# ZhenlongYuan/DVP-MVS

Hardware: AMD Instinct MI355X
Metric: Mpixels/sec/PatchMatch-iteration (higher is better)
Workload: dtype f32

## Files before the change

__graft_entry__.py:

```python
import importlib
import os
import subprocess
import sys

ROOT = os.path.dirname(os.path.abspath(__file__))
if ROOT not in sys.path:
    sys.path.insert(0, ROOT)


def build() -> None:
    subprocess.check_call(["make", "-s", "-C", os.path.join(ROOT, "dvp-mvs_amd", "csrc")])
    host = os.path.join(ROOT, "dvp-mvs_amd", "host")
    if os.path.exists(os.path.join(host, "Makefile")):
        subprocess.check_call(["make", "-s", "-C", host])
    subprocess.check_call(["make", "-s", "-C", os.path.join(ROOT, "oracle")])
    subprocess.check_call(["make", "-s", "-C", os.path.join(ROOT, "tests", "emul")])
    subprocess.check_call(["make", "-s", "-C", os.path.join(ROOT, "tests", "host")])
    subprocess.check_call(["make", "-s", "-C", os.path.join(ROOT, "tests", "half16")])
    subprocess.check_call(["make", "-s", "-C", os.path.join(ROOT, "tests", "jpeg_host")])
    pkg = importlib.import_module("dvp-mvs_amd")
    lib = pkg.get_capi().lib()
    missing = [s for s in pkg.get_capi().EXPORTS if not hasattr(lib, s)]
    if missing:
        raise RuntimeError("libdvp_mvs_hip.so lacks symbols: %s" % missing)


def smoke() -> None:
    import numpy as np
    pkg = importlib.import_module("dvp-mvs_amd")
    synth, capi = pkg.synth, pkg.get_capi()
    from oracle import oracle as O
    W, H, S = 96, 64, 3
    sc = synth.make_scene(W, H, S)
    p = synth.default_params(S + 1, max_iterations=1, state=synth.FIRST_INIT, use_APD=0)
    p["depth_min"] = np.float32(2.5) * np.float32(0.6)
    p["depth_max"] = np.float32(6.5) * np.float32(1.2)
    state = dict(planes=np.zeros((H * W, 4), np.float32), edge=sc["edge"], label=sc["label"],
                 radius=np.full(H * W, 5, np.int32))
    g = capi.from_scene(sc, p, device=0)
    g.upload_state(**state)
    g.run_patchmatch()
    o = O.from_scene(sc, p)
    o.upload_state(**state)
    o.run_patchmatch()
    pg, po = g.get("planes"), o.get("planes")
    same = (pg.view(np.uint32) == po.view(np.uint32)) | (np.isnan(pg) & np.isnan(po))
    if not same.all():
        raise AssertionError("smoke: HIP planes differ from the oracle in %d values" % int((~same).sum()))
    for n in ("selected_views", "weak_info", "radius"):
        if not (g.get(n) == o.get(n)).all():
            raise AssertionError("smoke: %s differs from the oracle" % n)
    print("smoke ok: %dx%d S=%d bit-exact vs oracle; total %.2f ms" % (W, H, S, g.timings()["total_ms"]))


if __name__ == "__main__":
    build()
    if os.path.exists("/dev/kfd"):
        smoke()
```

dvp-mvs_amd/csrc/dvp_engine.hip:

```cpp
#include "dvp_stages.hpp"
#include "dvp_jpeg_enc.h"
#include <hip/hip_runtime.h>
#include <cstdlib>
#include <string>
#include <vector>
#include <cstdio>
#include <cstring>
#include <mutex>
#include <condition_variable>
#include <thread>
#include <chrono>
#include <algorithm>
#include <cmath>

using namespace dvp;

struct LaunchArgs {
	int tiles_x, tiles, rows, half, colour, iter;
};

template <int STAGE, int SMP, int MV = 32>
__device__ __forceinline__ void stage_body(const Dev& d, const LaunchArgs& a) {
	const int lane = threadIdx.x & 63;
	const int wave = threadIdx.x >> 6;
// ... 140 lines not shown
	for (int i0 = 0; i0 < total; i0 += 64) {
		const bool valid = i0 + lane < total;
		const int i = valid ? i0 + lane : total - 1;
		const int pl = items[i];
		const int k = i - __shfl(off, pl, 64);
		uint32_t m = (uint32_t)__shfl((int)uniq, pl, 64);
		for (int j = 0; j < k; ++j) m &= m - 1;
		const int slot = dvp_ctz(m);
		PatchCtx ci;
		ci.tab = PatchTab{&lds_tab[pl], 64};
		ci.sum_ref = __shfl(c.sum_ref, pl, 64);
		ci.sum_ref_ref = __shfl(c.sum_ref_ref, pl, 64);
		ci.wsum = __shfl(c.wsum, pl, 64);
		ci.radius = __shfl(c.radius, pl, 64);
		ci.inc = __shfl(c.inc, pl, 64);
		ci.fast = __shfl(c.fast, pl, 64);
		const int ipx = __shfl(px, pl, 64), ipy = __shfl(py, pl, 64);
		strong_eval_item<SMP>(d, ci, ipx, ipy, slot, valid, d.eval_counter ? &cnt : nullptr);
	}
	if (d.eval_counter && cnt) atomicAdd(d.eval_counter, cnt);
}
extern "C" __global__ void __launch_bounds__(64, DVP_LB_HEAVY) dvp_strong_eval_items(const Dev d, const LaunchArgs a) { strong_eval_items_body<0>(d, a); }
extern "C" __global__ void __launch_bounds__(64, DVP_LB_HEAVY) dvp_strong_eval_items_exact(const Dev d, const LaunchArgs a) { strong_eval_items_body<1>(d, a); }
DVP_KERNEL64(dvp_strong_refine, kStageStrongRefine, DVP_LB_HEAVY)
DVP_KERNEL64(dvp_strong_refine_lanes, kStageStrongRefineLanes, DVP_LB_HEAVY)
template <int MV>
__device__ __forceinline__ void strong_decide_body(const Dev& d, const LaunchArgs& a) {
	int px, py;
	if (!block_to_pixel(blockIdx.x, threadIdx.x & 63, threadIdx.x >> 6, a.tiles_x, a.tiles, a.rows, a.half, a.colour, d.width, d.height, &px, &py)) return;
	if (d.weak_info[px + py * d.width] != DVP_WEAK) strong_decide_px<MV>(d, px, py, a.iter);
}
#ifndef DVP_LB_DECIDE
#define DVP_LB_DECIDE 4
#endif
#define DVP_DECIDE_KERNEL(MV) extern "C" __global__ void __launch_bounds__(256, DVP_LB_DECIDE) dvp_strong_decide_v##MV(const Dev d, const LaunchArgs a) { strong_decide_body<MV>(d, a); }
DVP_DECIDE_KERNEL(4)
DVP_DECIDE_KERNEL(6)
DVP_DECIDE_KERNEL(8)
DVP_DECIDE_KERNEL(10)
DVP_DECIDE_KERNEL(12)
DVP_DECIDE_KERNEL(16)
DVP_KERNEL(dvp_get_depth_normal, DVP_ST_GET_DEPTH_NORMAL, 1)
DVP_KERNEL(dvp_filter_strong, DVP_ST_FILTER_STRONG, 1)
DVP_KERNEL(dvp_depth_to_weak, DVP_ST_DEPTH_TO_WEAK, DVP_LB_HEAVY)
DVP_KERNEL(dvp_local_refine, DVP_ST_LOCAL_REFINE, DVP_LB_HEAVY)
DVP_KERNEL(dvp_depth_to_weak_refine, kStageSweeps, DVP_LB_HEAVY)
template <int WHAT>
__device__ __forceinline__ void sweep_light_body(const Dev& d, const LaunchArgs& a) {
	int px, py;
	if (!block_to_pixel(blockIdx.x, threadIdx.x & 63, threadIdx.x >> 6, a.tiles_x, a.tiles, a.rows, 0, 0, d.width, d.height, &px, &py)) return;
	if (WHAT != 0 && d.sweep_row1 > 0 && (py < d.sweep_row0 || py >= d.sweep_row1)) return;
	if (WHAT == 0) sweep_prepare_px(d, px, py);
	else if (WHAT == 1) sweep_decide1_px(d, px, py);
	else sweep_decide2_px(d, px, py);
}
extern "C" __global__ void __launch_bounds__(256) dvp_sweep_prepare(const Dev d, const LaunchArgs a) { sweep_light_body<0>(d, a); }
extern "C" __global__ void __launch_bounds__(256) dvp_sweep_decide1(const Dev d, const LaunchArgs a) { sweep_light_body<1>(d, a); }
extern "C" __global__ void __launch_bounds__(256) dvp_sweep_decide2(const Dev d, const LaunchArgs a) { sweep_light_body<2>(d, a); }
#ifndef DVP_SWEEP_ROWS
#define DVP_SWEEP_ROWS 14
#endif
constexpr int kSweepRows = DVP_SWEEP_ROWS;
template <int SMP>
__device__ __forceinline__ void sweep_eval_body(const Dev& d, const LaunchArgs& a) {
	const int lane = threadIdx.x;
	const int v = blockIdx.y;
	__shared__ f2 lds_tab[kTaps * kTaps * 64];
	__shared__ uint16_t list[64 * kSweepRows];
	__shared__ DvpCamera cams[2];
	const PatchTab tab{&lds_tab[lane], 64};
	static_assert(sizeof(DvpCamera) == 112, "28 dwords");
	if (lane < 56) {
		const int which = lane >= 28 ? 1 : 0;
		reinterpret_cast<uint32_t*>(&cams[which])[lane - 28 * which] = reinterpret_cast<const uint32_t*>(d.cameras + (which ? v + 1 : 0))[lane - 28 * which];
	}
	const int tiles_y = a.tiles / a.tiles_x;
	int tx, ty;
	{
		const int per_strip = 8 * tiles_y;
		const int st = (int)blockIdx.x / per_strip, rem = (int)blockIdx.x - st * per_strip;
		const int w_last = a.tiles_x - st * 8;
		if (w_last >= 8) { ty = rem >> 3; tx = st * 8 + (rem & 7); }
		else { ty = rem / w_last; tx = st * 8 + (rem - ty * w_last); }
	}
	ty += a.rows;
	const int x = tx * 64 + lane;
	int n = 0;
	for (int r = 0; r < kSweepRows; ++r) {
		const int y = ty * kSweepRows + r;
		const bool go = x < d.width && y < d.height && sweep_go(d, x + y * d.width, v, a.iter);
		const unsigned long long m = __ballot(go);
		if (go) list[n + __popcll(m & ((1ull << lane) - 1ull))] = (uint16_t)(r * 64 + lane);
		n += __popcll(m);
	}
	__syncthreads();
	unsigned long long cnt = 0;
	for (int i0 = 0; i0 < n; i0 += 64) {
		if (i0 + lane < n) {
			const int e = list[i0 + lane];
			sweep_eval_px<SMP>(d, tx * 64 + (e & 63), ty * kSweepRows + (e >> 6), v, a.iter, tab, d.eval_counter ? &cnt : nullptr, cams);
		}
	}
	if (d.eval_counter && cnt) atomicAdd(d.eval_counter, cnt);
}
template <int SMP>
__device__ __forceinline__ void sweep_border_body(const Dev& d, const LaunchArgs& a) {
	__shared__ f2 lds_tab[kTaps * kTaps * 64];
	const PatchTab tab{&lds_tab[threadIdx.x], 64};
	const int W = d.width, H = d.height;
	const long long t = (long long)blockIdx.x * 64 + threadIdx.x;
	int px, py;
	if (t < 12ll * W) {
		const int r = (int)(t / W);
		px = (int)(t - (long long)r * W);
		py = r < 6 ? r : H - 12 + r;
	} else {
		const long long u = t - 12ll * W;
		const int r = (int)(u / 12), cidx = (int)(u - 12ll * r);
		if (r >= H - 12) return;
		py = 6 + r;
		px = cidx < 6 ? cidx : W - 12 + cidx;
	}
	unsigned long long n = 0;
	run_pixel<kStageSweeps, SMP>(d, px, py, kSweepBorderOnly, d.eval_counter ? &n : nullptr, tab);
	if (d.eval_counter && n) atomicAdd(d.eval_counter, n);
}
extern "C" __global__ void __launch_bounds__(64, DVP_LB_HEAVY) dvp_sweep_border(const Dev d, const LaunchArgs a) { sweep_border_body<0>(d, a); }
extern "C" __global__ void __launch_bounds__(64, DVP_LB_HEAVY) dvp_sweep_border_exact(const Dev d, const LaunchArgs a) { sweep_border_body<1>(d, a); }
extern "C" __global__ void __launch_bounds__(64, DVP_LB_HEAVY) dvp_sweep_eval(const Dev d, const LaunchArgs a) { sweep_eval_body<0>(d, a); }
extern "C" __global__ void __launch_bounds__(64, DVP_LB_HEAVY) dvp_sweep_eval_exact(const Dev d, const LaunchArgs a) { sweep_eval_body<1>(d, a); }

DVP_KERNEL_LIST(dvp_find_nearest_strong_list, DVP_ST_FIND_NEAREST_STRONG, 1)
extern "C" __global__ void __launch_bounds__(256) dvp_gen_neighbours_list(const Dev d, const ListArgs a) {
	__shared__ s2 pts[kGnDirSlots * 256];
	const int t = list_block(blockIdx.x, gridDim.x, kListRun) * 256 + threadIdx.x;
	if (t >= a.count) return;
	const int center = d.weak_list[a.base + t];
	const int py = center / d.width, px = center - py * d.width;
	gen_neighbours_px(d, px, py, pts + threadIdx.x, 256);
}
DVP_KERNEL_LIST(dvp_neighbour_update_list, DVP_ST_NEIGHBOUR_UPDATE, 1)
DVP_KERNEL_LIST(dvp_ransac_fit_plane_list, DVP_ST_RANSAC_FIT, 1)
extern "C" __global__ void __launch_bounds__(64) dvp_ransac_fit_plane_wave(const Dev d, const ListArgs a) {
	__shared__ RansacShared sh[1];
	const int t = list_block(blockIdx.x, gridDim.x, kWaveRun * 4);
	if (t >= a.count) return;
	const int center = d.weak_list[a.base + t];
	const int py = center / d.width, px = center - py * d.width;
	ransac_fit_plane_wave(d, px, py, a.iter, sh[0]);
}

template <int SMP, int FMT, int TAB>
__device__ __forceinline__ void weak_wave_body(const Dev& d, const ListArgs& a) {
	__shared__ WeakSharedT<TAB> sh[1];
	const int wave = 0;
	const int t = list_block(blockIdx.x, gridDim.x, kWaveRun * 4);
	if (t >= a.count) return;
	const int center = d.weak_list[a.base + t];
	const int py = center / d.width, px = center - py * d.width;
	if (py >= a.covered_rows) return;
	if (d.weak_info[center] != DVP_WEAK) return;
	unsigned long long n = 0;
	weak_update_wave<SMP, FMT, TAB>(d, px, py, a.iter, d.eval_counter ? &n : nullptr, sh[wave]);
	if (d.eval_counter && n) atomicAdd(d.eval_counter, n);
}
#ifndef DVP_LB_GN
#define DVP_LB_GN 8
#endif
extern "C" __global__ void __launch_bounds__(256, DVP_LB_GN) dvp_gen_neighbours_search(const Dev d, const ListArgs a) {
	__shared__ GnShared sh[4];
	const int wave = threadIdx.x >> 6;
	const int t = list_block(blockIdx.x, gridDim.x, kWaveRun) * 4 + wave;
	if (t >= a.count) return;
	const int center = d.weak_list[a.base + t];
	if (d.weak_info[center] != DVP_WEAK) return;
	const int py = center / d.width, px = center - py * d.width;
	gen_neighbours_search_wave(d, px, py, sh[wave]);
}
extern "C" __global__ void __launch_bounds__(64, 3) dvp_gen_neighbours_fit(const Dev d, const ListArgs a) {
	__shared__ FitShared sh[1];
	const int wave = 0;
	const int t = list_block(blockIdx.x, gridDim.x, kWaveRun * 4);
	if (t >= a.count) return;
// ... 603 lines not shown
			float acc = 0.0f;
			for (int k = 0; k < 62; ++k) acc += tot[k];
			out[center] = acc;
		}
		__builtin_amdgcn_wave_barrier();
	}
}
extern "C" int dvp_probe(dvp_ctx* c, int mode, int K, int stride, int repeat, float* mean_ms, float* checksum);
#endif

struct EventPair { int stage; hipEvent_t a, b; };
enum { EV_TOTAL = -1, EV_ITER_LOOP = -2 };

struct dvp_ctx {
	int device = 0;
	int W = 0, H = 0, NI = 0, pitch = 0;
	size_t L = 0;
	hipStream_t stream = nullptr;
	int cand_mask_mode = -1;
	bool cand_mask_on = true;
	uint8_t* cand_mask = nullptr;
	unsigned *cand_list = nullptr, *cand_n = nullptr;
	uint32_t* sel_snap = nullptr;
	hipStream_t side = nullptr;
	hipEvent_t side_fork = nullptr, side_join = nullptr;
	Dev d{};
	std::vector<void*> allocs;
	float* images = nullptr;
	uint8_t* images8 = nullptr;
	int* images8_flag = nullptr;
	bool images8_ok = false;
	bool no_images8 = false;
	uint32_t* images16 = nullptr;
	bool images16_ok = false;
	bool no_images16 = false;
	float* image_stage = nullptr;
	float* depths = nullptr;
	uint32_t* edge_bits = nullptr;
	uint32_t* strong_bits = nullptr;
	uint32_t* strong_bits_t = nullptr;
	int* edge_sat = nullptr;
	DvpCamera* cameras = nullptr; ViewConst* views = nullptr; int* sector_taps = nullptr; int* sector_start = nullptr;
	f4* planes = nullptr; f4* planes_snap = nullptr; f4* fit_planes = nullptr;
	int* search_pos = nullptr;
	float* slot_costs = nullptr;
	float* strong_rec = nullptr;
	bool strong_split = true;
	bool eval_items = true;
	bool refine_lanes = true;
	f4* sweep_rec = nullptr; float* sweep_cost = nullptr; float* sweep_pc = nullptr;
	bool ransac_wave = false;
	bool sweep_split = true;
	bool sweep_force = false;
	double sweep_band_gb = 0.0;
	int sweep_band_rows = 0;
	bool gn_wave = false;
	float* costs = nullptr; float* costs_snap = nullptr; float* complex_ = nullptr;
	uint32_t* selected_views = nullptr;
	uint8_t* view_weight = nullptr; uint8_t* weak_info = nullptr; uint8_t* weak_reliable = nullptr; uint8_t* edge = nullptr;
	s2* label_stop = nullptr; s2* weak_nearest_strong = nullptr; s2* neighbours = nullptr; s2* gn_points = nullptr; int* gn_count = nullptr; s2* candidate = nullptr; s2* edge_neigh = nullptr; s2* label_boundary = nullptr;
	int* neighbours_map = nullptr; int* label = nullptr; int* radius = nullptr;
	unsigned long long* eval_counter = nullptr;
	float* scratch_out = nullptr;
	size_t weak_alloc = 0;
	AnchorRec* anchor_tab = nullptr;
	size_t anchor_tab_alloc = 0;
	bool anchor_tab_valid = false;
	bool anchor_tab_off = false;
	WeakRec* weak_rec = nullptr; f2* weak_ctab = nullptr; float* weak_ev = nullptr;
	size_t weak_phase_alloc = 0;
	bool weak_phased = true;
	int weak_phased_min = 8192;
	int weak_run[4] = { 64, 256, 1024, 1024 };
	int weak_group[4] = { 1, 4, 4, 2 };
	int* weak_list = nullptr;
	size_t weak_list_alloc = 0;
	int* weak_counts = nullptr;
	int* weak_totals_host = nullptr;
	uint8_t* coarse = nullptr;
	uint8_t* maps_out = nullptr;
	hipStream_t copy = nullptr;
	uint8_t* maps_host = nullptr;
	std::mutex dl_m;
	std::condition_variable dl_cv;
	bool dl_busy = false;
	bool dl_fetching = false;
	size_t coarse_alloc = 0;
	uint8_t* pv_bgr[3] = { nullptr, nullptr, nullptr };
	dvpjpeg::Encoder pv_enc[3];
	unsigned long long* pv_total = nullptr;
	hipEvent_t pv_done = nullptr;
	hipStream_t pv_copy = nullptr;
	int pv_kinds = 0;
	f4* saved_planes = nullptr; uint32_t* saved_views = nullptr; uint8_t* saved_weak = nullptr; int* saved_radius = nullptr;
	bool have_saved = false;
	int lut_radius = -1;
	bool have_depths = false;
	bool profiling = false;
	std::vector<EventPair> events;
	DvpTimings timings{};
	std::string error;
};

static std::string g_create_error;

#define HIP_TRY(ctx, expr)                                                                          \
// ... 36 lines not shown
	d.plane_stride = (size_t)c->pitch * (c->H + 2 * kImgPad);
	d.images = c->images; d.images8 = c->images8_ok ? c->images8 : nullptr; d.img8_tiles_x = img8_tiles_x(c->W); d.img8_plane_bytes = (size_t)img8_tiles_x(c->W) * img8_tiles_y(c->H) * 128;
	d.images16 = c->images16_ok ? c->images16 : nullptr; d.img16_tiles_x = img16_tiles_x(c->W); d.img16_plane_bytes = img16_plane_bytes(c->W, c->H);
	d.depths = c->depths; d.cameras = c->cameras; d.views = c->views; d.sector_taps = c->sector_taps; d.sector_start = c->sector_start;
	d.search_pos = c->search_pos;
	d.sweep_px0 = 0; d.sweep_row0 = 0; d.sweep_row1 = 0;
	d.sweep_rec = c->sweep_rec; d.sweep_cost = c->sweep_cost; d.sweep_pc = c->sweep_pc; d.slot_costs = c->slot_costs; d.strong_rec = c->strong_rec; d.half_w = (c->W + 1) / 2;
	d.planes = c->planes; d.planes_snap = c->planes_snap; d.costs = c->costs; d.costs_snap = c->costs_snap;
	d.selected_views = c->selected_views; d.view_weight = c->view_weight; d.weak_info = c->weak_info;
	d.weak_reliable = c->weak_reliable; d.weak_nearest_strong = c->weak_nearest_strong;
	d.anchor_tab = (c->anchor_tab_off || !c->anchor_tab_valid) ? nullptr : c->anchor_tab; d.neighbours_map = c->neighbours_map; d.neighbours = c->neighbours; d.gn_points = c->gn_points; d.gn_count = c->gn_count; d.fit_planes = c->fit_planes;
	d.candidate = c->candidate; d.edge = c->edge; d.edge_bits = c->edge_bits; d.strong_bits = c->strong_bits; d.strong_bits_t = c->strong_bits_t; d.edge_sat = c->edge_sat; d.sat_cells_x = sat_cells(c->W); d.sat_cells_y = sat_cells(c->H); d.edge_tiles_x = edge_tiles_x(c->W); d.edge_neigh = c->edge_neigh; d.label = c->label;
	d.label_boundary = c->label_boundary; d.label_stop = c->label_stop; d.complex_ = c->complex_; d.radius = c->radius;
	d.weak_list = c->weak_list;
	d.weak_rec = c->weak_rec; d.weak_ctab = c->weak_ctab; d.weak_ev = c->weak_ev;
	d.eval_counter = c->profiling ? c->eval_counter : nullptr;
}

static int ensure_images16(dvp_ctx* c) {
	if (c->images16) return 0;
	return dalloc(c, &c->images16, img16_plane_bytes(c->W, c->H) / 4 * c->NI, false);
}

static int set_device(dvp_ctx* c) {
	HIP_TRY(c, hipSetDevice(c->device));
	return 0;
}

extern "C" {

int dvp_ctx_create(int device, int width, int height, int num_images, dvp_ctx** out) {
	if (!out) return 1;
	*out = nullptr;
	if (width <= 0 || height <= 0 || num_images < 2 || num_images > DVP_MAX_IMAGES || width > 32767 || height > 32767) {
		g_create_error = "dvp_ctx_create: bad dimensions (2 <= num_images <= 32, sizes <= 32767: short2 pixel coordinates)";
		return 1;
	}
	{
		const unsigned long long pitch = ((unsigned long long)width + 2 * kImgPad + 63) / 64 * 64;
		if (pitch * ((unsigned long long)height + 2 * kImgPad) * 8ull >= (1ull << 32)) {
			g_create_error = "dvp_ctx_create: image too large (a padded row-pair plane must stay below 4 GiB)";
			return 1;
		}
	}
	dvp_ctx* c = new dvp_ctx();
	c->device = device; c->W = width; c->H = height; c->NI = num_images;
	c->no_images8 = getenv("DVP_NO_IMAGES8") != nullptr;
	c->no_images16 = getenv("DVP_NO_IMAGES16") != nullptr;
	if (const char* e = getenv("DVP_STRONG_SPLIT")) c->strong_split = atoi(e) != 0;
	if (const char* e = getenv("DVP_REFINE_LANES")) c->refine_lanes = atoi(e) != 0;
	if (const char* e = getenv("DVP_EVAL_ITEMS")) c->eval_items = atoi(e) != 0;
	if (const char* e = getenv("DVP_SWEEP_SPLIT")) { c->sweep_split = atoi(e) != 0; c->sweep_force = atoi(e) == 2; }
	if (const char* e = getenv("DVP_SWEEP_BAND_GB")) c->sweep_band_gb = atof(e);
	if (const char* e = getenv("DVP_WEAK_ANCHOR_TAB")) c->anchor_tab_off = atoi(e) == 0;
	if (const char* e = getenv("DVP_GN_WAVE")) c->gn_wave = atoi(e) != 0;
	if (const char* e = getenv("DVP_RANSAC_WAVE")) c->ransac_wave = atoi(e) != 0;
	if (const char* e = getenv("DVP_CAND_MASK")) c->cand_mask_mode = atoi(e) != 0 ? 1 : 0;
	if (const char* e = getenv("DVP_WEAK_PHASED")) c->weak_phased = atoi(e) != 0;
	if (const char* e = getenv("DVP_WEAK_PHASED_MIN")) c->weak_phased_min = atoi(e);
	if (const char* e = getenv("DVP_WEAK_RUNS")) {
		int g[4];
		if (sscanf(e, "%d,%d,%d,%d", &g[0], &g[1], &g[2], &g[3]) == 4)
			for (int i = 0; i < 4; ++i) c->weak_run[i] = g[i] < 1 ? 1 : g[i];
	}
	if (const char* e = getenv("DVP_WEAK_GROUPS")) {
		int g[4];
		if (sscanf(e, "%d,%d,%d,%d", &g[0], &g[1], &g[2], &g[3]) == 4)
			for (int i = 0; i < 4; ++i) c->weak_group[i] = g[i] < 1 ? 1 : (g[i] > kGrp ? kGrp : g[i]);
	}
	c->pitch = (width + 2 * kImgPad + 63) / 64 * 64;
	c->L = (size_t)width * height;
	auto fail = [&](int) { g_create_error = c->error; dvp_ctx_destroy(c); return 1; };
	if (set_device(c)) return fail(0);
	if (hipStreamCreateWithFlags(&c->stream, hipStreamNonBlocking) != hipSuccess) { c->error = "hipStreamCreate failed"; return fail(0); }
	if (hipStreamCreateWithFlags(&c->side, hipStreamNonBlocking) != hipSuccess || hipEventCreateWithFlags(&c->side_fork, hipEventDisableTiming) != hipSuccess ||
	    hipEventCreateWithFlags(&c->side_join, hipEventDisableTiming) != hipSuccess) { c->error = "hipStreamCreate failed"; return fail(0); }
	const size_t L = c->L, S = (size_t)num_images - 1, plane = (size_t)c->pitch * (height + 2 * kImgPad);
	int r = 0;
	r |= dalloc(c, &c->images, plane * num_images * 2);
	r |= dalloc(c, &c->images8, (size_t)img8_tiles_x(width) * img8_tiles_y(height) * 128 * num_images);
	r |= dalloc(c, &c->images8_flag, (size_t)1);
	r |= dalloc(c, &c->image_stage, plane * num_images);
	r |= dalloc(c, &c->cameras, (size_t)num_images);
	r |= dalloc(c, &c->views, (size_t)num_images);
	r |= dalloc(c, &c->planes, L);
	r |= dalloc(c, &c->planes_snap, L);
	r |= dalloc(c, &c->search_pos, L * 16);
	r |= dalloc(c, &c->fit_planes, L);
	r |= dalloc(c, &c->costs, L);
	r |= dalloc(c, &c->costs_snap, L);
	r |= dalloc(c, &c->selected_views, L + (size_t)width);
	r |= dalloc(c, &c->view_weight, L * 32);
	r |= dalloc(c, &c->weak_info, L);
	r |= dalloc(c, &c->weak_reliable, L);
	r |= dalloc(c, &c->weak_nearest_strong, L);
	r |= dalloc(c, &c->neighbours_map, L);
	r |= dalloc(c, &c->candidate, L * S * 8);
	r |= dalloc(c, &c->edge, L);
	r |= dalloc(c, &c->edge_bits, edge_bits_words(width, height));
	r |= dalloc(c, &c->strong_bits, edge_bits_words(width, height));
	r |= dalloc(c, &c->strong_bits_t, edge_bits_words(width, height));
	r |= dalloc(c, &c->edge_sat, (size_t)(sat_cells(width) + 1) * (sat_cells(height) + 1));
	r |= dalloc(c, &c->edge_neigh, L * 8);
	r |= dalloc(c, &c->label, L);
	r |= dalloc(c, &c->radius, L);
	r |= dalloc(c, &c->eval_counter, (size_t)1);
// ... 385 lines not shown
		if (t) (void)hipFree(t);
		c->weak_phased = false;
		fprintf(stderr, "dvp: no room for the phased weak update's hand-over buffers (%.2f GB); using the one-wave kernel\n", (double)cap * (sizeof(WeakRec) + 288 + 32 * S) / 1e9);
		sync_dev_struct(c);
		return 0;
	}
	c->allocs.push_back(r); c->allocs.push_back(t); c->allocs.push_back(e);
	c->weak_rec = (WeakRec*)r; c->weak_ctab = (f2*)t; c->weak_ev = (float*)e;
	c->weak_phase_alloc = cap;
	sync_dev_struct(c);
	return 0;
}

static void ensure_strong_split_buffers(dvp_ctx* c) {
	if (c->slot_costs || !c->strong_split || c->NI - 1 > 16) return;
	const size_t Lh = (size_t)((c->W + 1) / 2) * c->H;
	void *sc = nullptr, *sr = nullptr;
	if (getenv("DVP_TEST_SPLIT_ALLOC_FAIL")  || hipMalloc(&sc, (size_t)kSlotCount * (c->NI - 1) * Lh * sizeof(*c->slot_costs) + 64 ) != hipSuccess || hipMalloc(&sr, (size_t)SR_FIELDS * Lh * sizeof(*c->strong_rec)) != hipSuccess) {
		(void)hipGetLastError();
		if (sc) (void)hipFree(sc);
		c->strong_split = false;
		fprintf(stderr, "dvp: no room for the split strong update's cost buffer (%.1f GB); using the monolithic kernel\n", (double)kSlotCount * (c->NI - 1) * Lh * 4 / 1e9);
	} else {
		c->allocs.push_back(sc); c->allocs.push_back(sr);
		c->slot_costs = (decltype(c->slot_costs))sc; c->strong_rec = (decltype(c->strong_rec))sr;
		sync_dev_struct(c);
	}
}
static void ensure_sweep_buffers(dvp_ctx* c) {
	if (c->sweep_cost || !c->sweep_split) return;
	const size_t L = c->L;
	void *r = nullptr, *sc = nullptr, *pc = nullptr;
	size_t band_px = L;
	c->sweep_band_rows = 0;
	if (c->sweep_band_gb > 0.0) {
		const double whole = (double)sweep_cost_floats(L, c->NI - 1) * sizeof(float);
		const int bands = (int)std::ceil(whole / (c->sweep_band_gb * 1e9));
		if (bands > 1) {
			int rows = (c->H + bands - 1) / bands;
			rows = (rows + kSweepRows - 1) / kSweepRows * kSweepRows;
			if (rows < c->H) { c->sweep_band_rows = rows; band_px = (size_t)rows * c->W; }
		}
	}
	if (getenv("DVP_TEST_SWEEP_ALLOC_FAIL") || hipMalloc(&r, 2 * L * sizeof(f4)) != hipSuccess || hipMalloc(&pc, 61 * L * sizeof(float)) != hipSuccess ||
	    hipMalloc(&sc, sweep_cost_floats(band_px, c->NI - 1) * sizeof(float)) != hipSuccess) {
		(void)hipGetLastError();
		if (r) (void)hipFree(r);
		if (pc) (void)hipFree(pc);
		c->sweep_split = false;
		fprintf(stderr, "dvp: no room for the view-compacted DepthToWeak's cost buffer (%.1f GB); using the fused kernel\n", (double)(c->NI - 1) * kSweepFields * L * 4 / 1e9);
	} else {
		c->allocs.push_back(r); c->allocs.push_back(sc); c->allocs.push_back(pc);
		c->sweep_rec = (f4*)r; c->sweep_cost = (float*)sc; c->sweep_pc = (float*)pc;
		sync_dev_struct(c);
	}
}

static int launch_stage(dvp_ctx* c, int stage, int iter, int colour, bool fused = false) {
	if (stage < 0 || stage >= DVP_ST_LAUNCHABLE) { c->error = "bad stage id"; return 1; }
	if (!c->sector_taps) { c->error = "dvp_set_params must be called before running kernels"; return 1; }
	if (c->d.params.geom_consistency && !c->have_depths) { c->error = "geom_consistency is on but no depth maps were uploaded"; return 1; }
	const LaunchGeom g = make_geom(c->W, c->H, stage_is_half(stage));
	LaunchArgs a;
	a.tiles_x = g.tiles_x; a.tiles = g.tiles; a.rows = g.rows; a.half = g.half ? 1 : 0;
	a.colour = colour; a.iter = iter;
	if (c->events.size() >= 2048 && dvp_get_timings(c, nullptr)) return 1;
	if (stage != DVP_ST_STRONG_UPDATE && stage != DVP_ST_RANSAC_FIT && stage != DVP_ST_WEAK_UPDATE) c->anchor_tab_valid = false;
	if (stage == DVP_ST_STRONG_UPDATE) {
		EventPair prep;
		prep.stage = DVP_ST_STRONG_PREP;
		HIP_TRY(c, hipEventCreate(&prep.a));
		HIP_TRY(c, hipEventCreate(&prep.b));
		HIP_TRY(c, hipEventRecord(prep.a, c->stream));
		HIP_TRY(c, hipMemcpyAsync(c->planes_snap, c->planes, c->L * 16, hipMemcpyDeviceToDevice, c->stream));
		HIP_TRY(c, hipMemcpyAsync(c->costs_snap, c->costs, c->L * 4, hipMemcpyDeviceToDevice, c->stream));
		hipLaunchKernelGGL(dvp_strong_search, dim3(g.grid()), dim3(256), 0, c->stream, c->d, a);
		HIP_TRY(c, hipGetLastError());
		HIP_TRY(c, hipEventRecord(prep.b, c->stream));
		c->events.push_back(prep);
	}
	EventPair ep;
	ep.stage = stage;
	HIP_TRY(c, hipEventCreate(&ep.a));
	HIP_TRY(c, hipEventCreate(&ep.b));
	if (c->profiling) HIP_TRY(c, hipMemsetAsync(c->eval_counter, 0, 8, c->stream));
	HIP_TRY(c, hipEventRecord(ep.a, c->stream));
	const dim3 grid(g.grid()), block(256);
	const dim3 wave_grid((unsigned)((g.grid() + 7) / 8 * 32)), wave_block(64);
	const bool list_stage = stage == DVP_ST_FIND_NEAREST_STRONG || stage == DVP_ST_GEN_NEIGHBOURS || stage == DVP_ST_NEIGHBOUR_UPDATE ||
	                        stage == DVP_ST_RANSAC_FIT || stage == DVP_ST_WEAK_UPDATE;
	if (stage == DVP_ST_FIND_NEAREST_STRONG && c->d.weak_black + c->d.weak_red > 0) {
		const size_t words = edge_bits_words(c->W, c->H);
		hipLaunchKernelGGL(dvp_pack_edge_bits, dim3((unsigned)((words + 255) / 256)), dim3(256), 0, c->stream, c->weak_info, c->strong_bits, c->W, c->H, edge_tiles_x(c->W), words, (int)DVP_STRONG);
		hipLaunchKernelGGL(dvp_pack_bits_transposed, dim3((unsigned)((words + 255) / 256)), dim3(256), 0, c->stream, c->weak_info, c->strong_bits_t, c->W, c->H, edge_tiles_x(c->W), words, (int)DVP_STRONG);
		HIP_TRY(c, hipGetLastError());
	}
	if (stage == DVP_ST_GEN_NEIGHBOURS || stage == DVP_ST_RANSAC_FIT) {
		const size_t words = edge_bits_words(c->W, c->H);
		hipLaunchKernelGGL(dvp_pack_edge_bits, dim3((unsigned)((words + 255) / 256)), dim3(256), 0, c->stream, c->edge, c->edge_bits, c->W, c->H, edge_tiles_x(c->W), words, -1);
		HIP_TRY(c, hipGetLastError());
		const int cells = c->d.sat_cells_x * c->d.sat_cells_y;
		hipLaunchKernelGGL(dvp_edge_cell_counts, dim3((cells + 255) / 256), dim3(256), 0, c->stream, c->d);
		hipLaunchKernelGGL(dvp_edge_sat_rows, dim3((c->d.sat_cells_y + 1 + 63) / 64), dim3(64), 0, c->stream, c->d);
		hipLaunchKernelGGL(dvp_edge_sat_cols, dim3((c->d.sat_cells_x + 1 + 63) / 64), dim3(64), 0, c->stream, c->d);
		HIP_TRY(c, hipGetLastError());
		if (stage == DVP_ST_GEN_NEIGHBOURS) {
// ... 76 lines not shown
		}
		hipLaunchKernelGGL(c->d.sampler ? dvp_gen_edge_inform_exact : dvp_gen_edge_inform, grid, block, 0, c->stream, c->d, a);
		break;
	case DVP_ST_RANDOM_INIT: hipLaunchKernelGGL(c->d.sampler ? dvp_random_init_exact : dvp_random_init, grid, block, 0, c->stream, c->d, a); break;
	case DVP_ST_STRONG_UPDATE:
		if (c->strong_split && c->NI - 1 <= 16) {
			ensure_strong_split_buffers(c);
		}
		if (c->strong_split && c->NI - 1 <= 16) {
			const int S = c->NI - 1;
			if (c->eval_items) hipLaunchKernelGGL(c->d.sampler ? dvp_strong_eval_items_exact : dvp_strong_eval_items, wave_grid, wave_block, 0, c->stream, c->d, a);
			else hipLaunchKernelGGL(c->d.sampler ? dvp_strong_eval_exact : dvp_strong_eval, wave_grid, wave_block, 0, c->stream, c->d, a);
			if (S <= 4) hipLaunchKernelGGL(dvp_strong_decide_v4, grid, block, 0, c->stream, c->d, a);
			else if (S <= 6) hipLaunchKernelGGL(dvp_strong_decide_v6, grid, block, 0, c->stream, c->d, a);
			else if (S <= 8) hipLaunchKernelGGL(dvp_strong_decide_v8, grid, block, 0, c->stream, c->d, a);
			else if (S <= 10) hipLaunchKernelGGL(dvp_strong_decide_v10, grid, block, 0, c->stream, c->d, a);
			else if (S <= 12) hipLaunchKernelGGL(dvp_strong_decide_v12, grid, block, 0, c->stream, c->d, a);
			else hipLaunchKernelGGL(dvp_strong_decide_v16, grid, block, 0, c->stream, c->d, a);
			if (c->refine_lanes && (size_t)c->pitch * (c->H + 2 * kImgPad) * 8 * c->NI < ((size_t)1 << 32))
				hipLaunchKernelGGL(c->d.sampler ? dvp_strong_refine_lanes_exact : dvp_strong_refine_lanes, wave_grid, wave_block, 0, c->stream, c->d, a);
			else hipLaunchKernelGGL(c->d.sampler ? dvp_strong_refine_exact : dvp_strong_refine, wave_grid, wave_block, 0, c->stream, c->d, a);
		}
		else if (c->NI - 1 <= kNarrowViews) hipLaunchKernelGGL(c->d.sampler ? dvp_strong_update_v8_exact : dvp_strong_update_v8, grid, block, 0, c->stream, c->d, a);
		else if (c->NI - 1 <= 16) hipLaunchKernelGGL(c->d.sampler ? dvp_strong_update_v16_exact : dvp_strong_update_v16, grid, block, 0, c->stream, c->d, a);
		else hipLaunchKernelGGL(c->d.sampler ? dvp_strong_update_exact : dvp_strong_update, grid, block, 0, c->stream, c->d, a);
		break;
	case DVP_ST_GET_DEPTH_NORMAL: hipLaunchKernelGGL(c->d.sampler ? dvp_get_depth_normal_exact : dvp_get_depth_normal, grid, block, 0, c->stream, c->d, a); break;
	case DVP_ST_FILTER_STRONG: hipLaunchKernelGGL(c->d.sampler ? dvp_filter_strong_exact : dvp_filter_strong, grid, block, 0, c->stream, c->d, a); break;
	case DVP_ST_DEPTH_TO_WEAK: {
		const bool sweep_passes = fused && c->sweep_split && (c->d.params.geom_consistency || c->sweep_force);
		if (sweep_passes) ensure_sweep_buffers(c);
		if (sweep_passes && c->sweep_split) {
			const bool ex = c->d.sampler != 0;
			LaunchArgs s0 = a, s1 = a, sb = a;
			s0.iter = 0; s1.iter = 1; sb.iter = kSweepBorderOnly;
			const int etx = (c->W + 63) / 64, ety = (c->H + kSweepRows - 1) / kSweepRows;
			s0.tiles_x = s1.tiles_x = etx; s0.tiles = s1.tiles = etx * ety;
			const dim3 egrid((unsigned)(etx * ety), (unsigned)(c->NI - 1));
			hipLaunchKernelGGL(dvp_sweep_prepare, grid, block, 0, c->stream, c->d, a);
			const int band_rows = c->sweep_band_rows > 0 ? c->sweep_band_rows : c->H;
			for (int row0 = 0; row0 < c->H; row0 += band_rows) {
				Dev db = c->d;
				LaunchArgs b0 = s0, b1 = s1;
				dim3 bgrid = egrid;
				b0.rows = b1.rows = 0;
				if (c->sweep_band_rows > 0) {
					const int row1 = std::min(c->H, row0 + band_rows);
					db.sweep_px0 = row0 * c->W; db.sweep_row0 = row0; db.sweep_row1 = row1;
					const int bty = (row1 - row0 + kSweepRows - 1) / kSweepRows;
					b0.rows = b1.rows = row0 / kSweepRows;
					b0.tiles = b1.tiles = etx * bty;
					bgrid = dim3((unsigned)(etx * bty), (unsigned)(c->NI - 1));
				}
				hipLaunchKernelGGL(ex ? dvp_sweep_eval_exact : dvp_sweep_eval, bgrid, dim3(64), 0, c->stream, db, b0);
				hipLaunchKernelGGL(dvp_sweep_decide1, grid, block, 0, c->stream, db, a);
				if (sweep_window(c->d.params) < 30) {
					hipLaunchKernelGGL(ex ? dvp_sweep_eval_exact : dvp_sweep_eval, bgrid, dim3(64), 0, c->stream, db, b1);
				}
				hipLaunchKernelGGL(dvp_sweep_decide2, grid, block, 0, c->stream, db, a);
			}
			if (c->W >= 12 && c->H >= 12) {
				const long long frame = 12ll * c->W + 12ll * (c->H - 12);
				hipLaunchKernelGGL(ex ? dvp_sweep_border_exact : dvp_sweep_border, dim3((unsigned)((frame + 63) / 64)), dim3(64), 0, c->stream, c->d, sb);
			}
			else hipLaunchKernelGGL(ex ? dvp_depth_to_weak_refine_exact : dvp_depth_to_weak_refine, grid, block, 0, c->stream, c->d, sb);
		}
		else if (fused) hipLaunchKernelGGL(c->d.sampler ? dvp_depth_to_weak_refine_exact : dvp_depth_to_weak_refine, grid, block, 0, c->stream, c->d, a);
		else hipLaunchKernelGGL(c->d.sampler ? dvp_depth_to_weak_exact : dvp_depth_to_weak, grid, block, 0, c->stream, c->d, a);
		break;
	}
	case DVP_ST_LOCAL_REFINE: hipLaunchKernelGGL(c->d.sampler ? dvp_local_refine_exact : dvp_local_refine, grid, block, 0, c->stream, c->d, a); break;
	}
	HIP_TRY(c, hipGetLastError());
	}
	HIP_TRY(c, hipEventRecord(ep.b, c->stream));
	c->events.push_back(ep);
	if (c->profiling) {
		unsigned long long n = 0;
		HIP_TRY(c, hipMemcpyAsync(&n, c->eval_counter, 8, hipMemcpyDeviceToHost, c->stream));
		HIP_TRY(c, hipStreamSynchronize(c->stream));
		c->timings.ncc_evals[stage] += n;
	}
	return 0;
}

int dvp_run_stage(dvp_ctx* c, int stage, int iter, int colour) {
	if (set_device(c)) return 1;
	return launch_stage(c, stage, iter, colour);
}

int dvp_ctx_reserve(dvp_ctx* c, int weak_pixels, int flags) {
	if (set_device(c)) return 1;
	if (flags & 1) ensure_strong_split_buffers(c);
	if (flags & 2) ensure_sweep_buffers(c);
	if ((flags & 4) && !c->no_images8 && !c->no_images16 && ensure_images16(c)) return 1;
	if (weak_pixels > 0) {
		const size_t wc = std::min<size_t>((size_t)weak_pixels, c->L);
		if (grow_anchor_table(c, wc)) return 1;
		if (c->anchor_tab && grow_weak_phase_buffers(c, wc)) return 1;
		c->anchor_tab_valid = false;
	}
	return 0;
}

int dvp_synchronize(dvp_ctx* c) {
	if (set_device(c)) return 1;
	HIP_TRY(c, hipStreamSynchronize(c->stream));
	return 0;
}

int dvp_run_patchmatch(dvp_ctx* c) {
// ... 421 lines not shown
```

dvp-mvs_amd/csrc/dvp_strong.hpp:

```cpp
#ifndef DVP_STRONG_HPP_
#define DVP_STRONG_HPP_

#include "dvp_ncc.hpp"

namespace dvp {

DVP_HD void sort_small(float* v, int n) {
	for (int i = 1; i < n; i++) {
		const float tmp = v[i];
		int j = i;
		for (; j >= 1 && tmp < v[j - 1]; j--) v[j] = v[j - 1];
		v[j] = tmp;
	}
}

DVP_HD f4 random_normal_yzl_sel(const Dev& d, int px, int py, Rng& rng, float depth, uint32_t sel) {
	const int W = d.width, H = d.height;
	const DvpCamera rc = load_camera(d, 0);
	f3 vd[20];
	{
		const f4 v0 = view_direction(rc, px, py, depth);
		vd[0] = mk3(v0.x, v0.y, v0.z);
	}
	int index = 1;
// ... 1163 lines not shown
}
DVP_HD size_t sweep_cost_index(const Dev& d, int v, int f, int center) {
#if DVP_SWEEP_LAYOUT == 1
	const int S = d.params.num_images - 1;
	const int rel = center - d.sweep_px0;
	return (((size_t)(rel >> 6) * S + v) * kSweepFields + (size_t)f) * 64 + (size_t)(rel & 63);
#else
	const size_t L = (size_t)d.width * (size_t)d.height;
	return ((size_t)v * kSweepFields + (size_t)f) * L + (size_t)center;
#endif
}
DVP_HD bool sweep_is_border(const Dev& d, int px, int py) { return px < 6 || py < 6 || px >= d.width - 6 || py >= d.height - 6; }

DVP_HD void sweep_prepare_px(const Dev& d, int px, int py) {
	const int W = d.width;
	const int center = px + py * W;
	const size_t L = (size_t)W * (size_t)d.height;
	const DvpParams& P = d.params;
	const DvpCamera rc = load_camera(d, 0);
	const int S = P.num_images - 1;
	if (P.use_radius && d.radius[center] == 0) d.radius[center] = P.strong_radius;
	f4 info = mk4(0.0f, 0.0f, 0.0f, 0.0f);
	d.sweep_rec[L + center] = info;
	if (sweep_is_border(d, px, py)) { d.weak_info[center] = DVP_UNKNOWN; return; }
	const f4 origin = normal_world_to_cam(rc, d.planes[center]);
	if (origin.w == 0) { d.weak_info[center] = DVP_UNKNOWN; return; }
	const uint32_t sel = d.selected_views[center];
	const uint8_t* vw = d.view_weight + (size_t)center * 32;
	float base_line = 0, weight_normal = 0.0f;
	int valid = 0;
	for (int v = 0; v < S; ++v) {
		if (!is_set(sel, v)) continue;
		weight_normal += vw[v];
		const float c0 = rc.c[0] - d.cameras[v + 1].c[0];
		const float c1 = rc.c[1] - d.cameras[v + 1].c[1];
		const float c2 = rc.c[2] - d.cameras[v + 1].c[2];
		base_line += sqrtf(c0 * c0 + c1 * c1 + c2 * c2);
		valid++;
	}
	if (valid == 0) { d.weak_info[center] = DVP_UNKNOWN; return; }
	base_line /= valid;
	const float disp = rc.K[0] * base_line / origin.w;
	d.sweep_rec[center] = origin;
	d.sweep_rec[L + center] = mk4(base_line, disp, weight_normal, (float)(SWF_VALID | (weight_normal != 0 ? SWF_REFINE : 0)));
}

DVP_HD bool sweep_go(const Dev& d, int center, int v, int stage) {
	const size_t L = (size_t)d.width * (size_t)d.height;
	const int flags = (int)d.sweep_rec[L + center].w;
	if (!(flags & (stage == 0 ? SWF_VALID : SWF_PEAK))) return false;
	return is_set(d.selected_views[center], v) && d.view_weight[(size_t)center * 32 + v] != 0;
}

template <int SMP>
DVP_HD void sweep_eval_px(const Dev& d, int px, int py, int v, int stage, PatchTab tab, unsigned long long* nevals, const DvpCamera* cams = nullptr) {
	const int W = d.width;
	const int center = px + py * W;
	const size_t L = (size_t)W * (size_t)d.height;
	const DvpParams& P = d.params;
	const DvpCamera rc_own = load_camera(d, 0);
	const DvpCamera& rc = cams ? cams[0] : rc_own;
	const f4 origin = d.sweep_rec[center];
	const f4 info = d.sweep_rec[L + center];
	const float base_line = info.x, disp = info.y;
	const bool refine = ((int)info.w & SWF_REFINE) != 0;
	PatchCtx c;
	{
		int radius, inc;
		patch_geometry(d, center, &radius, &inc);
#if defined(DVP_ABL_SWEEP_NO_TABLE)
		c.tab = tab; c.radius = radius; c.inc = inc; c.fast = 1; c.sum_ref = 1.0f; c.sum_ref_ref = 2.0f; c.wsum = 1.0f;
		for (int t = 0; t < kTaps * kTaps; ++t) tab.set(t, mk2(d.nb_cos, d.nb_sin * (float)t));
#else
		build_patch_ctx(d, px, py, radius, inc, 0, tab, &c);
#endif
	}
	const int cw = sweep_window(P);
	float* out = d.sweep_cost + sweep_cost_index(d, v, 0, center);
	const size_t FS = sweep_field_stride(d);
	const int k0 = stage == 0 ? 0 : 2 * cw + 1, k1 = stage == 0 ? 2 * cw + 1 + (refine ? 1 : 0) : 61;
	for (int k = k0; k < k1; ++k) {
		const bool extra = stage == 0 && k == 2 * cw + 1;
		const int pd = k <= 2 * cw ? k - cw : (k - (2 * cw + 1) < 30 - cw ? k - (2 * cw + 1) - 30 : k - 30);
		float p_depth = origin.w;
		if (!extra) {
			p_depth = rc.K[0] * base_line / (disp + pd);
			if (p_depth < P.depth_min || p_depth > P.depth_max) continue;
		}
		f4 pl = origin;
		pl.w = distance_to_origin(rc, px, py, p_depth, pl);
		GeomFetch gf;
		const bool split_geom = P.geom_consistency && cams != nullptr;
#if !defined(DVP_ABL_SWEEP_NO_GEOM) && !defined(DVP_SWEEP_GEOM_AFTER)
		if (split_geom) gf = geom_cost_fetch(d, cams[0], cams[1], v + 1, px, py, pl);
#endif
#if defined(DVP_ABL_SWEEP_NO_EVAL)
		const float ncc = pl.w * 1e-3f;
#else
		const float ncc = ncc_old<SMP>(d, c, px, py, v + 1, pl);
#endif
		if (nevals) *nevals += 1;
#if defined(DVP_ABL_SWEEP_NO_GEOM)
		const float gc = 0.0f;
#elif defined(DVP_SWEEP_GEOM_AFTER)
		const float gc = !P.geom_consistency ? 0.0f : (cams ? geom_cost_cams(d, cams[0], cams[1], v + 1, px, py, pl) : geom_cost(d, px, py, v + 1, pl));
#else
		const float gc = !P.geom_consistency ? 0.0f : (split_geom ? geom_cost_finish(cams[0], cams[1], px, py, gf) : geom_cost(d, px, py, v + 1, pl));
#endif
#if defined(DVP_ABL_SWEEP_NO_STORE)
		if (ncc + gc != d.nb_thresh * 1e30f) continue;
#endif
		if (extra) {
			float t = ncc;
			if (P.geom_consistency) t += P.geom_factor * gc;
			DVP_NT_STORE(1, &out[(size_t)kSweepExtra * FS], t);
		} else if (pd >= -5 && pd <= 5) {
			DVP_NT_STORE(1, &out[(size_t)(pd + 30) * FS], ncc);
			if (P.geom_consistency) DVP_NT_STORE(1, &out[(size_t)(61 + pd + 5) * FS], gc);
		} else {
			float cst = ncc;
			if (P.geom_consistency) cst += P.geom_factor * gc;
			DVP_NT_STORE(1, &out[(size_t)(pd + 30) * FS], cst);
		}
	}
}

DVP_HD void sweep_fold(const Dev& d, int center, int pd, uint32_t sel, const uint8_t* vw, bool both, float* pc_out, float* lr_out) {
	const DvpParams& P = d.params;
	const int S = P.num_images - 1;
	const size_t FS = sweep_field_stride(d);
	float pc = 0.0f, lr = 0.0f;
	for (int v = 0; v < S; ++v) {
		if (!is_set(sel, v)) continue;
		if (vw[v] == 0) continue;
		const float* in = d.sweep_cost + sweep_cost_index(d, v, 0, center);
		float ncc = 0.0f, gc = 0.0f, cst;
		if (pd >= -5 && pd <= 5) {
			ncc = DVP_NT_LOAD(2, &in[(size_t)(pd + 30) * FS]);
			cst = ncc;
			if (P.geom_consistency) { gc = DVP_NT_LOAD(2, &in[(size_t)(61 + pd + 5) * FS]); cst += P.geom_factor * gc; }
		} else {
			cst = DVP_NT_LOAD(2, &in[(size_t)(pd + 30) * FS]);
		}
// ... 218 lines not shown
```

Before: 59.55.

## Split sweep evaluation into NCC-only pass and separate per-pixel geometric cost pass

Geometric-consistency cost is moved out of the heavy per-view sweep eval kernel. A new light kernel runs once per pixel and loops over all views, batching three views' projections and depth texel fetches. The NCC kernel now only writes raw NCC, and the geom pass reads it back and adds the weighted geometric term. This takes the geometry fetch latency and register pressure off the heavy kernel, at the cost of an extra launch and an extra read-modify-write of the cost volume.

```diff
diff --git a/__graft_entry__.py b/__graft_entry__.py
--- a/__graft_entry__.py
+++ b/__graft_entry__.py
@@ -15,6 +15,7 @@
         subprocess.check_call(["make", "-s", "-C", host])
     subprocess.check_call(["make", "-s", "-C", os.path.join(ROOT, "oracle")])
     subprocess.check_call(["make", "-s", "-C", os.path.join(ROOT, "tests", "emul")])
+    subprocess.check_call(["make", "-s", "-C", os.path.join(ROOT, "tests", "sweep_once")])
     subprocess.check_call(["make", "-s", "-C", os.path.join(ROOT, "tests", "host")])
     subprocess.check_call(["make", "-s", "-C", os.path.join(ROOT, "tests", "half16")])
     subprocess.check_call(["make", "-s", "-C", os.path.join(ROOT, "tests", "jpeg_host")])
diff --git a/dvp-mvs_amd/csrc/dvp_engine.hip b/dvp-mvs_amd/csrc/dvp_engine.hip
--- a/dvp-mvs_amd/csrc/dvp_engine.hip
+++ b/dvp-mvs_amd/csrc/dvp_engine.hip
@@ -216,25 +216,28 @@
 	if (WHAT != 0 && d.sweep_row1 > 0 && (py < d.sweep_row0 || py >= d.sweep_row1)) return;
 	if (WHAT == 0) sweep_prepare_px(d, px, py);
 	else if (WHAT == 1) sweep_decide1_px(d, px, py);
-	else sweep_decide2_px(d, px, py);
+	else if (WHAT == 2) sweep_decide2_px(d, px, py);
+	else sweep_geom_px(d, px, py, a.iter);
 }
 extern "C" __global__ void __launch_bounds__(256) dvp_sweep_prepare(const Dev d, const LaunchArgs a) { sweep_light_body<0>(d, a); }
 extern "C" __global__ void __launch_bounds__(256) dvp_sweep_decide1(const Dev d, const LaunchArgs a) { sweep_light_body<1>(d, a); }
 extern "C" __global__ void __launch_bounds__(256) dvp_sweep_decide2(const Dev d, const LaunchArgs a) { sweep_light_body<2>(d, a); }
+extern "C" __global__ void __launch_bounds__(256) dvp_sweep_geom(const Dev d, const LaunchArgs a) { sweep_light_body<3>(d, a); }
 #ifndef DVP_SWEEP_ROWS
 #define DVP_SWEEP_ROWS 14
 #endif
 constexpr int kSweepRows = DVP_SWEEP_ROWS;
-template <int SMP>
+template <int SMP, int PRE = 0>
 __device__ __forceinline__ void sweep_eval_body(const Dev& d, const LaunchArgs& a) {
 	const int lane = threadIdx.x;
 	const int v = blockIdx.y;
 	__shared__ f2 lds_tab[kTaps * kTaps * 64];
 	__shared__ uint16_t list[64 * kSweepRows];
-	__shared__ DvpCamera cams[2];
+	constexpr int kCams = PRE ? 1 : 2;
+	__shared__ DvpCamera cams[kCams];
 	const PatchTab tab{&lds_tab[lane], 64};
 	static_assert(sizeof(DvpCamera) == 112, "28 dwords");
-	if (lane < 56) {
+	if (lane < 28 * kCams) {
 		const int which = lane >= 28 ? 1 : 0;
 		reinterpret_cast<uint32_t*>(&cams[which])[lane - 28 * which] = reinterpret_cast<const uint32_t*>(d.cameras + (which ? v + 1 : 0))[lane - 28 * which];
 	}
@@ -262,7 +265,7 @@
 	for (int i0 = 0; i0 < n; i0 += 64) {
 		if (i0 + lane < n) {
 			const int e = list[i0 + lane];
-			sweep_eval_px<SMP>(d, tx * 64 + (e & 63), ty * kSweepRows + (e >> 6), v, a.iter, tab, d.eval_counter ? &cnt : nullptr, cams);
+			sweep_eval_px<SMP, PRE>(d, tx * 64 + (e & 63), ty * kSweepRows + (e >> 6), v, a.iter, tab, d.eval_counter ? &cnt : nullptr, cams);
 		}
 	}
 	if (d.eval_counter && cnt) atomicAdd(d.eval_counter, cnt);
@@ -293,6 +296,8 @@
 extern "C" __global__ void __launch_bounds__(64, DVP_LB_HEAVY) dvp_sweep_border_exact(const Dev d, const LaunchArgs a) { sweep_border_body<1>(d, a); }
 extern "C" __global__ void __launch_bounds__(64, DVP_LB_HEAVY) dvp_sweep_eval(const Dev d, const LaunchArgs a) { sweep_eval_body<0>(d, a); }
 extern "C" __global__ void __launch_bounds__(64, DVP_LB_HEAVY) dvp_sweep_eval_exact(const Dev d, const LaunchArgs a) { sweep_eval_body<1>(d, a); }
+extern "C" __global__ void __launch_bounds__(64, DVP_LB_HEAVY) dvp_sweep_eval_ncc(const Dev d, const LaunchArgs a) { sweep_eval_body<0, kSweepGeomAfter>(d, a); }
+extern "C" __global__ void __launch_bounds__(64, DVP_LB_HEAVY) dvp_sweep_eval_ncc_exact(const Dev d, const LaunchArgs a) { sweep_eval_body<1, kSweepGeomAfter>(d, a); }
 
 DVP_KERNEL_LIST(dvp_find_nearest_strong_list, DVP_ST_FIND_NEAREST_STRONG, 1)
 extern "C" __global__ void __launch_bounds__(256) dvp_gen_neighbours_list(const Dev d, const ListArgs a) {
@@ -1002,6 +1007,9 @@
 	bool ransac_wave = false;
 	bool sweep_split = true;
 	bool sweep_force = false;
+	size_t sweep_cost_bytes = 0;
+	bool sweep_poison = false;
+	bool sweep_geom_pass = true;
 	double sweep_band_gb = 0.0;
 	int sweep_band_rows = 0;
 	bool gn_wave = false;
@@ -1144,6 +1152,8 @@
 	if (const char* e = getenv("DVP_EVAL_ITEMS")) c->eval_items = atoi(e) != 0;
 	if (const char* e = getenv("DVP_SWEEP_SPLIT")) { c->sweep_split = atoi(e) != 0; c->sweep_force = atoi(e) == 2; }
 	if (const char* e = getenv("DVP_SWEEP_BAND_GB")) c->sweep_band_gb = atof(e);
+	if (const char* e = getenv("DVP_SWEEP_GEOM_PASS")) c->sweep_geom_pass = atoi(e) != 0;
+	c->sweep_poison = getenv("DVP_TEST_SWEEP_POISON") != nullptr;
 	if (const char* e = getenv("DVP_WEAK_ANCHOR_TAB")) c->anchor_tab_off = atoi(e) == 0;
 	if (const char* e = getenv("DVP_GN_WAVE")) c->gn_wave = atoi(e) != 0;
 	if (const char* e = getenv("DVP_RANSAC_WAVE")) c->ransac_wave = atoi(e) != 0;
@@ -1635,6 +1645,7 @@
 	} else {
 		c->allocs.push_back(r); c->allocs.push_back(sc); c->allocs.push_back(pc);
 		c->sweep_rec = (f4*)r; c->sweep_cost = (float*)sc; c->sweep_pc = (float*)pc;
+		c->sweep_cost_bytes = sweep_cost_floats(band_px, c->NI - 1) * sizeof(float);
 		sync_dev_struct(c);
 	}
 }
@@ -1817,11 +1828,20 @@
 					b0.tiles = b1.tiles = etx * bty;
 					bgrid = dim3((unsigned)(etx * bty), (unsigned)(c->NI - 1));
 				}
-				hipLaunchKernelGGL(ex ? dvp_sweep_eval_exact : dvp_sweep_eval, bgrid, dim3(64), 0, c->stream, db, b0);
+				if (c->sweep_poison) HIP_TRY(c, hipMemsetAsync(c->sweep_cost, 0xFF, c->sweep_cost_bytes, c->stream));
+				const bool gp = c->sweep_geom_pass && c->d.params.geom_consistency;
+				LaunchArgs g0 = a, g1 = a;
+				g0.iter = 0; g1.iter = 1;
+				auto evaluate = [&](const LaunchArgs& ea, const LaunchArgs& ga) {
+					if (gp) {
+						hipLaunchKernelGGL(ex ? dvp_sweep_eval_ncc_exact : dvp_sweep_eval_ncc, bgrid, dim3(64), 0, c->stream, db, ea);
+						hipLaunchKernelGGL(dvp_sweep_geom, grid, block, 0, c->stream, db, ga);
+					}
+					else hipLaunchKernelGGL(ex ? dvp_sweep_eval_exact : dvp_sweep_eval, bgrid, dim3(64), 0, c->stream, db, ea);
+				};
+				evaluate(b0, g0);
 				hipLaunchKernelGGL(dvp_sweep_decide1, grid, block, 0, c->stream, db, a);
-				if (sweep_window(c->d.params) < 30) {
-					hipLaunchKernelGGL(ex ? dvp_sweep_eval_exact : dvp_sweep_eval, bgrid, dim3(64), 0, c->stream, db, b1);
-				}
+				if (sweep_window(c->d.params) < 30) evaluate(b1, g1);
 				hipLaunchKernelGGL(dvp_sweep_decide2, grid, block, 0, c->stream, db, a);
 			}
 			if (c->W >= 12 && c->H >= 12) {
diff --git a/dvp-mvs_amd/csrc/dvp_strong.hpp b/dvp-mvs_amd/csrc/dvp_strong.hpp
--- a/dvp-mvs_amd/csrc/dvp_strong.hpp
+++ b/dvp-mvs_amd/csrc/dvp_strong.hpp
@@ -1239,7 +1239,73 @@
 	return is_set(d.selected_views[center], v) && d.view_weight[(size_t)center * 32 + v] != 0;
 }
 
-template <int SMP>
+constexpr int kSweepGeomViews = 3;
+DVP_HD void sweep_geom_px(const Dev& d, int px, int py, int stage) {
+	const int W = d.width;
+	const int center = px + py * W;
+	const size_t L = (size_t)W * (size_t)d.height;
+	const DvpParams& P = d.params;
+	const f4 info = d.sweep_rec[L + center];
+	const int flags = (int)info.w;
+	if (!(flags & (stage == 0 ? SWF_VALID : SWF_PEAK))) return;
+	const int S = P.num_images - 1;
+	const uint32_t sel = d.selected_views[center];
+	const uint8_t* vw = d.view_weight + (size_t)center * 32;
+	uint32_t go = 0;
+	for (int v = 0; v < S; ++v)
+		if (is_set(sel, v) && vw[v] != 0) go |= 1u << v;
+	if (go == 0) return;
+	const DvpCamera rc = load_camera(d, 0);
+	const f4 origin = d.sweep_rec[center];
+	const float base_line = info.x, disp = info.y;
+	const bool refine = (flags & SWF_REFINE) != 0;
+	const int cw = sweep_window(P);
+	const size_t FS = sweep_field_stride(d);
+	const int k0 = stage == 0 ? 0 : 2 * cw + 1, k1 = stage == 0 ? 2 * cw + 1 + (refine ? 1 : 0) : 61;
+	for (int k = k0; k < k1; ++k) {
+		const bool extra = stage == 0 && k == 2 * cw + 1;
+		const int pd = k <= 2 * cw ? k - cw : (k - (2 * cw + 1) < 30 - cw ? k - (2 * cw + 1) - 30 : k - 30);
+		float p_depth = origin.w;
+		if (!extra) {
+			p_depth = rc.K[0] * base_line / (disp + pd);
+			if (p_depth < P.depth_min || p_depth > P.depth_max) continue;
+		}
+		f4 pl = origin;
+		pl.w = distance_to_origin(rc, px, py, p_depth, pl);
+		const f3 fwd = geom_forward_point(d, px, py, pl);
+		const bool alone = !extra && pd >= -5 && pd <= 5;
+		const int field = extra ? kSweepExtra : (alone ? 61 + pd + 5 : pd + 30);
+		for (int v0 = 0; v0 < S; v0 += kSweepGeomViews) {
+			if (wave_all(((go >> v0) & ((1u << kSweepGeomViews) - 1u)) == 0)) continue;
+			GeomFetch gf[kSweepGeomViews];
+			float ncc[kSweepGeomViews];
+#pragma unroll
+			for (int j = 0; j < kSweepGeomViews; ++j) {
+				const int v = v0 + j < S ? v0 + j : S - 1;
+				const DvpCamera sc = load_camera(d, v + 1);
+				float sd;
+				project_on_camera(fwd, sc, &gf[j].sp, &sd);
+				const float cx = fminf(fmaxf(gf[j].sp.x, -1.0f), (float)d.width);
+				const float cy = fminf(fmaxf(gf[j].sp.y, -1.0f), (float)d.height);
+				gf[j].src_depth = tex_texel(d.depths + (size_t)(v + 1) * d.plane_stride, d.org, d.pitch, d.width, d.height, (int)cx, (int)cy);
+				ncc[j] = 0.0f;
+				if (!alone) ncc[j] = DVP_NT_LOAD(2, &d.sweep_cost[sweep_cost_index(d, v, field, center)]);
+			}
+			sched_fence();
+#pragma unroll
+			for (int j = 0; j < kSweepGeomViews; ++j) {
+				const int v = v0 + j;
+				if (v >= S || !((go >> v) & 1u)) continue;
+				const float gc = geom_cost_finish(rc, load_camera(d, v + 1), px, py, gf[j]);
+				DVP_NT_STORE(1, &d.sweep_cost[sweep_cost_index(d, v, field, center)], alone ? gc : ncc[j] + P.geom_factor * gc);
+			}
+		}
+	}
+}
+
+enum { kSweepGeomAfter = 1 };
+
+template <int SMP, int PRE = 0>
 DVP_HD void sweep_eval_px(const Dev& d, int px, int py, int v, int stage, PatchTab tab, unsigned long long* nevals, const DvpCamera* cams = nullptr) {
 	const int W = d.width;
 	const int center = px + py * W;
@@ -1276,6 +1342,12 @@
 		}
 		f4 pl = origin;
 		pl.w = distance_to_origin(rc, px, py, p_depth, pl);
+		if (PRE & kSweepGeomAfter) {
+			const float ncc = ncc_old<SMP>(d, c, px, py, v + 1, pl);
+			if (nevals) *nevals += 1;
+			DVP_NT_STORE(1, &out[(size_t)(extra ? kSweepExtra : pd + 30) * FS], ncc);
+			continue;
+		}
 		GeomFetch gf;
 		const bool split_geom = P.geom_consistency && cams != nullptr;
 #if !defined(DVP_ABL_SWEEP_NO_GEOM) && !defined(DVP_SWEEP_GEOM_AFTER)
```

After: 58.79. -1.3%, worse.
